# yzhang511/multi_modal_foundation_model

Measured on AMD Instinct MI355X. Metric: pretrain samples/sec (T=100 bins/modality, d_model=256, 5+5 layers, spike+behaviour masked pretraining step), higher is better.
Workload: dtype bf16; 1 GPU; BASELINE.json configs[1]: 1 session, ap(668 neurons)+behaviour(2), d_model=256, heads=8, mlp=512, 5 enc + 5 dec layers, T=100 (L=200 tokens), dropout 0.4/0.2, AdamW+OneCycleLR, mixed objectives; per_gpu_batch=1024, global_batch=1024, seq_len=200, parallelism=dp1

## Files before the change

### multi_modal_foundation_model_amd/csrc/attention_fast.hip

```cpp
#include "attn_common.h"
#include "attn_route.h"
#include <algorithm>
#include <stdlib.h>

using namespace attn;

namespace {

constexpr int KEEP_BITS = 10;

struct KeepArgs {
    uint32_t* bits;
    const uint32_t* state;
    uint32_t site, thresh;
    uint32_t nwords;
    int nkt, Lk;
};
__global__ __launch_bounds__(256) void attn_keepbits_kernel(const KeepArgs a) {
    const uint32_t gid = blockIdx.x * 256u + threadIdx.x;
    if (gid >= a.nwords) return;
    const uint32_t w = gid & 31u, kt = (gid >> 5) % (uint32_t)a.nkt;
    if ((int)(32u * kt + ((w >> 1) & 3u) + 8u * (w >> 3) + 4u * (w & 1u)) >= a.Lk) return;
    const uint32_t k0 = mix32(a.state[0] + a.site * 0x9E3779B9u), k1 = mix32(a.state[1] ^ (a.site * 0x85EBCA6Bu + 0xC2B2AE35u));
    const uint32_t s = mix32(gid ^ k0);
    const uint32_t kb = k1 + __umul24(s >> 24, 0x9E3779u);
    uint32_t r = 0;
#pragma unroll
    for (int j = 0; j < KEEP_BITS; ++j) {
        if ((a.thresh & ((2u << j) - 1u)) == 0) continue;
        uint32_t h = __umul24(s + (uint32_t)j * 0x3C6EF35Fu, 0x7FEB35u) + kb;
        h ^= h >> 13;
        h = __umul24(h, 0x46CA6Bu);
        h ^= h >> 16;
        r = ((a.thresh >> j) & 1u) ? (h | r) : (h & r);
    }
    a.bits[gid] = r;
}

__device__ __forceinline__ void stage_mod(uint8_t* modb, int* tmod, int t, int LP, uint32_t mv) {
    const int lane = t & 63;
    if (t < LP) modb[t] = (uint8_t)mv;
    const uint32_t first = (uint32_t)__shfl((int)mv, lane & 32);
    const uint64_t eq = __ballot(mv == first);
    const uint32_t half = (lane & 32) ? (uint32_t)(eq >> 32) : (uint32_t)eq;
    if ((lane & 31) == 0 && (t >> 5) < 8) tmod[t >> 5] = half == 0xffffffffu ? (int)mv : TMOD_MIXED;
}
template <int G, bool DROP>
__device__ __forceinline__ void fwd_tile(const f32x16& st, float c2, float nm, float& l_run, f32x16& acc, const Masks16& mk, const char* Vs,
                                         int kt, int lane) {
    uint32_t pk[8];
    float ps0 = 0.f, ps1 = 0.f;
#pragma unroll
    for (int r = 0; r < 16; r += 2) {
        if (r < 4 * G) {
            float p0 = __builtin_amdgcn_exp2f(__builtin_fmaf(st[r], c2, nm));
            float p1 = __builtin_amdgcn_exp2f(__builtin_fmaf(st[r + 1], c2, nm));
            ps0 = v_add(ps0, p0);
            ps1 = v_add(ps1, p1);
            if (DROP) {
                p0 = v_keep(p0, mk.m[r]);
                p1 = v_keep(p1, mk.m[r + 1]);
            }
            asm volatile("" : "+v"(p0), "+v"(p1), "+v"(ps0), "+v"(ps1));
            pk[r >> 1] = pack2(p0, p1);
        } else {
            pk[r >> 1] = 0u;
        }
    }
    l_run = v_add(l_run, v_add(ps0, ps1));
    const uint4 lo = make_uint4(pk[0], pk[1], pk[2], pk[3]), hi = make_uint4(pk[4], pk[5], pk[6], pk[7]);
    acc = __builtin_amdgcn_mfma_f32_32x32x16_bf16(trfrag(Vs, 64, kt * 32, 0, lane), __builtin_bit_cast(bf16x8v, lo), acc, 0, 0, 0);
    if (G > 2) acc = __builtin_amdgcn_mfma_f32_32x32x16_bf16(trfrag(Vs, 64, kt * 32 + 16, 0, lane), __builtin_bit_cast(bf16x8v, hi), acc, 0, 0, 0);
}
template <int G>
__device__ __forceinline__ float tile_max(const f32x16& st) {
    float mx = fmaxf(fmaxf(st[0], st[1]), st[2]);
#pragma unroll
    for (int r = 3; r < 4 * G; ++r) mx = fmaxf(mx, st[r]);
    return xhalf_max(mx);
}

constexpr int F_KRS = 80, F_VRS = 64, F_ORS = 80, F_MAXKT = 7;
constexpr float F_OVERFLOW = 1.2676506e30f;

template <int NW, bool DROP, int NKT, bool MASKED>
__global__ __launch_bounds__(NW * 64, 4) void attn_fwd_fast_kernel(const mmfm_attn_desc d, const float keep_scale) {
    constexpr int NT = NW * 64;
    extern __shared__ __attribute__((aligned(16))) char smem[];
    const int t = threadIdx.x, lane = t & 63, kh = lane >> 5, l31 = lane & 31;
    const int wave = __builtin_amdgcn_readfirstlane(t >> 6);
    const int bh_ = attn_xcd_remap((int)blockIdx.x, (int)gridDim.x, d.flags);
    const int b = bh_ / d.heads, h = bh_ % d.heads;
    const int Lq = d.Lq, Lk = d.Lk, LkP = NKT ? NKT * 32 : (Lk + 31) & ~31;
    const int nqt = (Lq + 31) >> 5, nkt = NKT ? NKT : LkP >> 5;
    char* Ks = smem;
    char* Vs = Ks + LkP * F_KRS;
    float* kbias = reinterpret_cast<float*>(Vs + LkP * F_VRS);
    char* ost = reinterpret_cast<char*>(kbias + LkP);
    int* wflag = reinterpret_cast<int*>(ost + NW * 32 * F_ORS);
    int* tmod = wflag + 8;
    float* kzero = reinterpret_cast<float*>(wflag + 16);
    uint8_t* modb = reinterpret_cast<uint8_t*>(kzero + LkP);
    const bool causal = MASKED && (d.flags & MMFM_ATTN_CAUSAL), sep = MASKED && (d.flags & MMFM_ATTN_SEP);
    const uint16_t* qg = reinterpret_cast<const uint16_t*>(d.q) + (size_t)b * Lq * d.ldq + h * 32;
    const uint16_t* kg = reinterpret_cast<const uint16_t*>(d.k) + (size_t)b * Lk * d.ldk + h * 32;
    const uint16_t* vg = reinterpret_cast<const uint16_t*>(d.v) + (size_t)b * Lk * d.ldv + h * 32;

    const int qt = wave;
    const int q0 = qt * 32, q = q0 + l31;
    uint4 kc[2], vc[2], qv[2];
    uint8_t kpv = 1;
#pragma unroll
    for (int j = 0; j < 2; ++j) {
        const int c = t + NT * j, row = c >> 2, col = c & 3;
        kc[j] = make_uint4(0u, 0u, 0u, 0u); vc[j] = kc[j];
        if (row < Lk) {
            kc[j] = *reinterpret_cast<const uint4*>(kg + (size_t)row * d.ldk + 8 * col);
            vc[j] = *reinterpret_cast<const uint4*>(vg + (size_t)row * d.ldv + 8 * col);
        }
    }
#pragma unroll
    for (int ks = 0; ks < 2; ++ks) {
        qv[ks] = make_uint4(0u, 0u, 0u, 0u);
        if (qt < nqt && q < Lq) qv[ks] = *reinterpret_cast<const uint4*>(qg + (size_t)q * d.ldq + ks * 16 + 8 * kh);
    }
    if (t < Lk && d.keypad != nullptr) kpv = d.keypad[(size_t)b * Lk + t];
    uint32_t mv = 0u;
    if constexpr (MASKED) {
        if (sep && t < LkP) mv = d.mod_id[min(t, Lk - 1)];
    }
#pragma unroll
    for (int j = 0; j < 2; ++j) {
        const int c = t + NT * j, row = c >> 2, col = c & 3;
        if (row < LkP) {
            *reinterpret_cast<uint4*>(Ks + row * F_KRS + col * 16) = kc[j];
            *reinterpret_cast<uint4*>(Vs + row * F_VRS + col * 16) = vc[j];
        }
    }
    const bool kok = t < Lk && (kpv != 0 || causal);
    if (t < LkP) kbias[t] = kok ? 0.f : -INFINITY;
    if constexpr (MASKED) {
        if (t < LkP) kzero[t] = t < Lk ? 0.f : -INFINITY;
        stage_mod(modb, tmod, t, LkP, mv);
    }
    const int pad = (t < Lk && !kok) ? 1 : 0;
    const int wv = __any(pad) ? 1 : 0;
    if (lane == 0) wflag[wave] = wv;
    __syncthreads();
    int anypad = 0;
#pragma unroll
    for (int w = 0; w < NW; ++w) anypad |= wflag[w];
    anypad = __builtin_amdgcn_readfirstlane(anypad);
    if (qt >= nqt) return;

    bf16x8v qf[2];
    qf[0] = __builtin_bit_cast(bf16x8v, qv[0]);
    qf[1] = __builtin_bit_cast(bf16x8v, qv[1]);
    const float c2 = d.scale * LOG2E;
    const bool fixdiag = anypad && (d.flags & MMFM_ATTN_DIAG);
    const masks_ptr mkp = reinterpret_cast<masks_ptr>(reinterpret_cast<uintptr_t>(d.keepbits)) + ((size_t)bh_ * nqt + qt) * nkt;
    int m_skip = 0, m_zero = 0, m_mix = 0, nkt_run = nkt;
    if constexpr (MASKED) {
        const int tq = sep ? tmod[qt] : 0;
        nkt_run = 1;
        for (int kt = 0; kt < nkt; ++kt) {
            const int c = tile_class(causal, sep, tq, sep ? tmod[kt] : 0, qt, kt);
            m_skip |= (c == T_SKIP) << kt;
            m_zero |= (c == T_ZERO) << kt;
            m_mix |= (c == T_MIXED) << kt;
            if (c != T_SKIP) nkt_run = kt + 1;
        }
        m_skip = __builtin_amdgcn_readfirstlane(m_skip);
        m_zero = __builtin_amdgcn_readfirstlane(m_zero);
        m_mix = __builtin_amdgcn_readfirstlane(m_mix);
        nkt_run = __builtin_amdgcn_readfirstlane(nkt_run);
    }
    auto skipped = [&](int kt) { return MASKED && ((m_skip >> kt) & 1); };

    auto score = [&](int kt) {
        const bool dfix = fixdiag && kt == qt;
        const float* bias = kbias;
        if constexpr (MASKED) bias = ((m_zero >> kt) & 1) ? kzero : kbias;
        f32x16 a;
#pragma unroll
        for (int g = 0; g < 4; ++g) {
            const float4 kb4 = *reinterpret_cast<const float4*>(bias + kt * 32 + 8 * g + 4 * kh);
            a[4 * g + 0] = kb4.x; a[4 * g + 1] = kb4.y; a[4 * g + 2] = kb4.z; a[4 * g + 3] = kb4.w;
        }
        if (dfix) {
            asm volatile("" ::: "memory");
#pragma unroll
            for (int r = 0; r < 16; ++r) a[r] = (mrow(r, kh) == l31) ? 0.f : a[r];
        }
        if constexpr (MASKED) {
            if ((m_mix >> kt) & 1) {
                asm volatile("" ::: "memory");
                const int fl = d.flags;
                const uint32_t mq = sep ? modb[q] : 0u;
#pragma unroll
                for (int g = 0; g < 4; ++g) {
                    const uint32_t mw = sep ? *reinterpret_cast<const uint32_t*>(modb + kt * 32 + 8 * g + 4 * kh) : 0u;
#pragma unroll
                    for (int i = 0; i < 4; ++i)
                        a[4 * g + i] = mixed_start(fl, q, kt * 32 + 8 * g + 4 * kh + i, Lk, a[4 * g + i], mq, (mw >> (8 * i)) & 0xffu);
                }
            }
        }
#pragma unroll
        for (int ks = 0; ks < 2; ++ks)
            a = __builtin_amdgcn_mfma_f32_32x32x16_bf16(rowfrag(Ks, (kt * 32 + l31) * F_KRS + ks * 32 + kh * 16), qf[ks], a, 0, 0, 0);
        return a;
    };
    const int gtail = ((Lk - (nkt - 1) * 32) + 7) >> 3;
    float m_ref, l_run = 0.f;
    f32x16 acc;
#pragma unroll
    for (int r = 0; r < 16; ++r) acc[r] = 0.f;
    auto tile = [&](int kt, const f32x16& st, const Masks16& mk) {
        if (kt == nkt - 1 && gtail != 4) {
            if (gtail == 1) fwd_tile<1, DROP>(st, c2, -m_ref, l_run, acc, mk, Vs, kt, lane);
            else if (gtail == 2) fwd_tile<2, DROP>(st, c2, -m_ref, l_run, acc, mk, Vs, kt, lane);
            else fwd_tile<3, DROP>(st, c2, -m_ref, l_run, acc, mk, Vs, kt, lane);
        } else {
            fwd_tile<4, DROP>(st, c2, -m_ref, l_run, acc, mk, Vs, kt, lane);
        }
    };
    {
        Masks16 mk[2];
        f32x16 sc[2];
        if (DROP) mk[0] = ld_masks(mkp);
        sc[0] = score(0);
        m_ref = v_max((nkt == 1 && gtail != 4) ? (gtail == 1 ? tile_max<1>(sc[0]) : gtail == 2 ? tile_max<2>(sc[0]) : tile_max<3>(sc[0]))
                                                : tile_max<4>(sc[0]), -1e30f / c2) * c2;
#pragma unroll
        for (int kt = 0; kt < F_MAXKT; ++kt) {
            if constexpr (!MASKED) {
                if (kt + 1 < nkt) {
                    sc[(kt + 1) & 1] = score(kt + 1);
                    if (DROP) mk[(kt + 1) & 1] = ld_masks(mkp + (kt + 1));
                }
                tile(kt, sc[kt & 1], mk[kt & 1]);
                if (kt + 1 >= nkt) break;
            } else {
                if (kt + 1 < nkt_run && !skipped(kt + 1)) {
                    sc[(kt + 1) & 1] = score(kt + 1);
                    if (DROP) mk[(kt + 1) & 1] = ld_masks(mkp + (kt + 1));
                }
                if (!skipped(kt)) tile(kt, sc[kt & 1], mk[kt & 1]);
                if (kt + 1 >= nkt_run) break;
            }
        }
    }
    float l_tot = xhalf_sum(l_run);
    if (__any(!(l_tot < F_OVERFLOW))) {
        float m_run = -1e30f;
        l_run = 0.f;
#pragma unroll
        for (int r = 0; r < 16; ++r) acc[r] = 0.f;
        for (int kt = 0; kt < nkt_run; ++kt) {
            if (skipped(kt)) continue;
            const f32x16 st = score(kt);
            Masks16 mk;
            if (DROP) mk = ld_masks(mkp + kt);
            const float mt = tile_max<4>(st) * c2;
            const float m_new = v_max(m_run, mt);
            const float alpha = __builtin_amdgcn_exp2f(m_run - m_new);
#pragma unroll
            for (int r = 0; r < 16; ++r) acc[r] *= alpha;
            l_run *= alpha;
            m_run = m_new;
            m_ref = m_run;
            tile(kt, st, mk);
        }
        l_tot = xhalf_sum(l_run);
    }
    const mmfm_attn_desc* kd = (const mmfm_attn_desc*)__builtin_amdgcn_kernarg_segment_ptr();
    asm volatile("" : "+s"(kd));
    const Drop dout = drop_init(kd->drop_o);
    const float inv = keep_scale / l_tot;
    if (kh == 0 && q < Lq) kd->lse[(size_t)bh_ * Lq + q] = m_ref * LN2 + __logf(l_tot);
    char* tl = ost + wave * 32 * F_ORS;
    const int heads = kd->heads, ldo = kd->ldo;
    uint16_t* og = reinterpret_cast<uint16_t*>(kd->o) + (size_t)b * Lq * ldo + h * 32;
    const uint64_t base = ((uint64_t)b * Lq + (uint64_t)q) * (uint64_t)(heads * 32) + (uint64_t)(h * 32);
#pragma unroll
    for (int g = 0; g < 4; ++g) {
        const int d0 = 8 * g + 4 * kh;
        float v0 = acc[4 * g + 0] * inv, v1 = acc[4 * g + 1] * inv, v2 = acc[4 * g + 2] * inv, v3 = acc[4 * g + 3] * inv;
        if (dout.on()) {
            dout.apply2(v0, v1, base + d0);
            dout.apply2(v2, v3, base + d0 + 2);
        }
        typedef __attribute__((ext_vector_type(4))) __bf16 bf16x4v;
        bf16x4v pk;
        pk[0] = (__bf16)v0; pk[1] = (__bf16)v1; pk[2] = (__bf16)v2; pk[3] = (__bf16)v3;
        *reinterpret_cast<uint2*>(tl + l31 * F_ORS + d0 * 2) = __builtin_bit_cast(uint2, pk);
    }
    wave_lds_fence();
#pragma unroll
    for (int i = 0; i < 2; ++i) {
        const int idx = lane + 64 * i, row = idx >> 2, c = idx & 3;
        if (q0 + row < Lq)
            *reinterpret_cast<uint4*>(og + (size_t)(q0 + row) * ldo + 8 * c) = *reinterpret_cast<const uint4*>(tl + row * F_ORS + c * 16);
    }
}

size_t fwd_fast_lds(int Lk, int nw, bool masked) {
    const int LkP = (Lk + 31) & ~31;
    return (size_t)LkP * (F_KRS + F_VRS + 4) + (size_t)nw * 32 * F_ORS + 64 + (masked ? (size_t)LkP * 5 : 0);
}

constexpr int B_NW = 8, B_CW = 7, B_TS = 80, B_TILE = 32 * B_TS, B_RS = 64, B_QRS = 80;

__device__ __forceinline__ int img_off(int row, int chunk) { return row * B_RS + ((chunk ^ ((row >> 2) & 3)) << 4); }
__device__ __forceinline__ bf16x8v trfrag_sw(const char* S, int rbase, int lane) {
    const int g = lane >> 4, li = lane & 15, q = li >> 2, p = li & 3;
    const int r0 = 4 * (g >> 1) + q;
    const int chunk = 2 * (g & 1) + (p >> 1), byte = 8 * (p & 1);
    const s16x4 lo = __builtin_amdgcn_ds_read_tr16_b64_v4i16((lds_s16x4*)(S + (rbase + r0) * B_RS + ((chunk ^ (g >> 1)) << 4) + byte));
    const s16x4 hi = __builtin_amdgcn_ds_read_tr16_b64_v4i16((lds_s16x4*)(S + (rbase + r0 + 8) * B_RS + ((chunk ^ ((g >> 1) + 2)) << 4) + byte));
    s16x8 v;
    v[0] = lo[0]; v[1] = lo[1]; v[2] = lo[2]; v[3] = lo[3]; v[4] = hi[0]; v[5] = hi[1]; v[6] = hi[2]; v[7] = hi[3];
    return __builtin_bit_cast(bf16x8v, v);
}

template <int GRP, bool DROP>
__device__ __forceinline__ void bwd_tile(const f32x16& s, const f32x16& dpv, float c2, const float* lse2, const float* dl, uint32_t wsh,
                                         const char* As, const char* Bs, char* slot, int qt, int kh, int lane, f32x16& dKt, f32x16& dVt) {
#pragma unroll
    for (int s2 = 0; s2 < 2; ++s2) {
        if (2 * s2 >= GRP) continue;
        const bool both = GRP > 2 * s2 + 1;
        float pd[8], ds[8];
        const int qb = qt * 32 + 16 * s2 + 4 * kh;
#pragma unroll
        for (int e4 = 0; e4 < 2; ++e4) {
            if (e4 == 1 && !both) {
#pragma unroll
                for (int e = 4; e < 8; ++e) { pd[e] = 0.f; ds[e] = 0.f; }
                continue;
            }
            const float4 l4 = *reinterpret_cast<const float4*>(lse2 + qb + 8 * e4), d4 = *reinterpret_cast<const float4*>(dl + qb + 8 * e4);
            const float lq[4] = {l4.x, l4.y, l4.z, l4.w}, dq_[4] = {d4.x, d4.y, d4.z, d4.w};
#pragma unroll
            for (int i = 0; i < 4; ++i) {
                const int e = 4 * e4 + i, r = 8 * s2 + e;
                const float p = __builtin_amdgcn_exp2f(__builtin_fmaf(s[r], c2, -lq[i]));
                float pm = p;
                if (DROP) {
                    int m = __builtin_amdgcn_sbfe((int)wsh, (r & 3) + 8 * (r >> 2), 1);
                    asm volatile("" : "+v"(m));
                    pm = __uint_as_float(__float_as_uint(p) & (uint32_t)m);
                }
                pd[e] = pm;
                ds[e] = __builtin_fmaf(pm, dpv[r], -v_mul(p, dq_[i]));
            }
        }
        const bf16x8v pf = pack8(pd), sf = pack8(ds);
        const uint4 sw = __builtin_bit_cast(uint4, sf);
        *reinterpret_cast<uint2*>(slot + (16 * s2 + 4 * kh) * 2) = make_uint2(sw.x, sw.y);
        *reinterpret_cast<uint2*>(slot + (16 * s2 + 8 + 4 * kh) * 2) = make_uint2(sw.z, sw.w);
        dVt = __builtin_amdgcn_mfma_f32_32x32x16_bf16(trfrag_sw(Bs, qt * 32 + 16 * s2, lane), pf, dVt, 0, 0, 0);
        dKt = __builtin_amdgcn_mfma_f32_32x32x16_bf16(trfrag_sw(As, qt * 32 + 16 * s2, lane), sf, dKt, 0, 0, 0);
    }
    if (GRP <= 2) {
        *reinterpret_cast<uint2*>(slot + (16 + 4 * kh) * 2) = make_uint2(0u, 0u);
        *reinterpret_cast<uint2*>(slot + (24 + 4 * kh) * 2) = make_uint2(0u, 0u);
    }
}

template <bool DROP, int NQT, bool MASKED>
__global__ __launch_bounds__(B_NW * 64, 4) void attn_bwd_fast_kernel(const mmfm_attn_desc d, const float keep_scale) {
    constexpr int NW = B_NW, CW = B_CW, TS = B_TS, TILE = B_TILE, RS = B_RS, NT = NW * 64;
    extern __shared__ __attribute__((aligned(16))) char smem[];
    const int t = threadIdx.x, lane = t & 63, kh = lane >> 5, l31 = lane & 31;
    const int wave = __builtin_amdgcn_readfirstlane(t >> 6);
    const int bh_ = attn_xcd_remap((int)blockIdx.x, (int)gridDim.x, d.flags);
    const int b = bh_ / d.heads, h = bh_ % d.heads;
    const int Lq = d.Lq, Lk = d.Lk, LqP = NQT ? NQT * 32 : (Lq + 31) & ~31, LkP = NQT ? NQT * 32 : (Lk + 31) & ~31;
    const int nqt = NQT ? NQT : LqP / 32, nkt = ((Lk + 31) & ~31) / 32;
    char* As = smem;
    char* Bs = As + LqP * RS;
    float* lse2 = reinterpret_cast<float*>(Bs + LqP * RS);
    float* dl = lse2 + LqP;
    float* kbias = dl + LqP;
    char* stg = reinterpret_cast<char*>(kbias + LkP);
    char* sc7 = stg + 2 * CW * TILE;
    uint32_t* flags = reinterpret_cast<uint32_t*>(sc7 + 32 * B_QRS);
    int* tmod = reinterpret_cast<int*>(flags + 8);
    uint8_t* modb = reinterpret_cast<uint8_t*>(flags + 16);
    const bool causal = MASKED && (d.flags & MMFM_ATTN_CAUSAL), sep = MASKED && (d.flags & MMFM_ATTN_SEP);
    const uint16_t* qg = reinterpret_cast<const uint16_t*>(d.q) + (size_t)b * Lq * d.ldq + h * 32;
    const uint16_t* kg = reinterpret_cast<const uint16_t*>(d.k) + (size_t)b * Lk * d.ldk + h * 32;
    const uint16_t* vg = reinterpret_cast<const uint16_t*>(d.v) + (size_t)b * Lk * d.ldv + h * 32;
    const uint16_t* og = reinterpret_cast<const uint16_t*>(d.o) + (size_t)b * Lq * d.ldo + h * 32;
    const uint16_t* dog = reinterpret_cast<const uint16_t*>(d.d_o) + (size_t)b * Lq * d.lddo + h * 32;
    const float osc_dk = d.scale * keep_scale, osc_dv = keep_scale, inv_keep = 1.f / keep_scale;
    const Drop dout = drop_init(d.drop_o);

    const int kt_own = wave < CW ? wave : 0, key_own = kt_own * 32 + l31;
    uint4 qc[2], kc[2], gc[2], oc[2], kfv[2], vfv[2];
#pragma unroll
    for (int j = 0; j < 2; ++j) {
        const int c = t + NT * j, row = c >> 2, col = c & 3;
        qc[j] = make_uint4(0u, 0u, 0u, 0u); kc[j] = qc[j]; gc[j] = qc[j]; oc[j] = qc[j];
        if (row < Lq) {
            qc[j] = *reinterpret_cast<const uint4*>(qg + (size_t)row * d.ldq + 8 * col);
            gc[j] = *reinterpret_cast<const uint4*>(dog + (size_t)row * d.lddo + 8 * col);
            oc[j] = *reinterpret_cast<const uint4*>(og + (size_t)row * d.ldo + 8 * col);
        }
        if (row < Lk) kc[j] = *reinterpret_cast<const uint4*>(kg + (size_t)row * d.ldk + 8 * col);
    }
#pragma unroll
    for (int ks = 0; ks < 2; ++ks) {
        kfv[ks] = make_uint4(0u, 0u, 0u, 0u); vfv[ks] = kfv[ks];
        if (wave < CW && key_own < Lk) {
            kfv[ks] = *reinterpret_cast<const uint4*>(kg + (size_t)key_own * d.ldk + ks * 16 + 8 * kh);
            vfv[ks] = *reinterpret_cast<const uint4*>(vg + (size_t)key_own * d.ldv + ks * 16 + 8 * kh);
        }
    }
    const uint32_t* kbp = reinterpret_cast<const uint32_t*>(d.keepbits) + ((size_t)bh_ * nqt * nkt + min(kt_own, nkt - 1)) * 32 +
                          2 * ((l31 & 3) + 4 * (l31 >> 3)) + ((l31 >> 2) & 1);
    const int kw_stride = nkt * 32;
    uint32_t kw_next = 0u;
    if (DROP) kw_next = kbp[0];
    float lsev = 0.f;
    uint8_t kpv = 1;
    if (t < Lq) lsev = d.lse[(size_t)bh_ * Lq + t];
    if (t < Lk && d.keypad != nullptr) kpv = d.keypad[(size_t)b * Lk + t];
    uint32_t mv = 0u;
    if constexpr (MASKED) {
        if (sep && t < LqP) mv = d.mod_id[min(t, Lq - 1)];
    }
#pragma unroll
    for (int j = 0; j < 2; ++j) {
        const int c = t + NT * j, row = c >> 2, col = c & 3;
        if (row < LqP) {
            *reinterpret_cast<uint4*>(As + img_off(row, col)) = qc[j];
            const uint32_t gw[4] = {gc[j].x, gc[j].y, gc[j].z, gc[j].w}, ow[4] = {oc[j].x, oc[j].y, oc[j].z, oc[j].w};
            const uint64_t base = ((uint64_t)b * Lq + (uint64_t)row) * (uint64_t)(d.heads * 32) + (uint64_t)(h * 32 + 8 * col);
            float part = 0.f, gd[8];
#pragma unroll
            for (int i = 0; i < 4; ++i) {
                float g0 = __uint_as_float(gw[i] << 16), g1 = __uint_as_float(gw[i] & 0xffff0000u);
                const float o0 = __uint_as_float(ow[i] << 16), o1 = __uint_as_float(ow[i] & 0xffff0000u);
                part += g0 * o0 + g1 * o1;
                if (dout.on()) dout.apply2(g0, g1, base + 2 * i);
                gd[2 * i] = g0;
                gd[2 * i + 1] = g1;
            }
            part += __shfl_xor(part, 1);
            part += __shfl_xor(part, 2);
            if (col == 0) dl[row] = part * inv_keep;
            *reinterpret_cast<uint4*>(Bs + img_off(row, col)) = __builtin_bit_cast(uint4, pack8(gd));
        }
        if (row < LkP) *reinterpret_cast<uint4*>(stg + img_off(row, col)) = kc[j];
    }
    if (t < LqP) lse2[t] = lsev * LOG2E;
    const bool kok = t < Lk && (kpv != 0 || causal);
    if (t < LkP) kbias[t] = kok ? 0.f : -INFINITY;
    if constexpr (MASKED) stage_mod(modb, tmod, t, LqP, mv);
    const int pad = (t < Lk && !kok) ? 1 : 0;
    const int wv = __any(pad) ? 1 : 0;
    if (lane == 0) flags[wave] = (uint32_t)wv;
    __syncthreads();
    int anypad = 0;
#pragma unroll
    for (int w = 0; w < NW; ++w) anypad |= (int)flags[w];
    anypad = __builtin_amdgcn_readfirstlane(anypad);
    const float c2 = d.scale * LOG2E;

    if (wave < CW) {
        const int kt = wave;
        const bool active = kt < nkt;
        f32x16 dKt, dVt;
#pragma unroll
        for (int r = 0; r < 16; ++r) { dKt[r] = 0.f; dVt[r] = 0.f; }
        const int key = kt * 32 + l31;
        bf16x8v kfr[2], vfr[2];
#pragma unroll
        for (int ks = 0; ks < 2; ++ks) {
            kfr[ks] = __builtin_bit_cast(bf16x8v, kfv[ks]);
            vfr[ks] = __builtin_bit_cast(bf16x8v, vfv[ks]);
        }
        const float kbv = active ? kbias[key] : 0.f;
        f32x16 s, dpv;
        int m_skip = 0, m_zero = 0, m_mix = 0;
        if constexpr (MASKED) {
            if (active) {
                const int tk = sep ? tmod[kt] : 0;
                for (int qt = 0; qt < nqt; ++qt) {
                    const int c = tile_class(causal, sep, sep ? tmod[qt] : 0, tk, qt, kt);
                    m_skip |= (c == T_SKIP) << qt;
                    m_zero |= (c == T_ZERO) << qt;
                    m_mix |= (c == T_MIXED) << qt;
                }
            }
            m_skip = __builtin_amdgcn_readfirstlane(m_skip);
            m_zero = __builtin_amdgcn_readfirstlane(m_zero);
            m_mix = __builtin_amdgcn_readfirstlane(m_mix);
        }
        const int roff0 = l31 * RS + (((0 + kh) ^ ((l31 >> 2) & 3)) << 4), roff1 = l31 * RS + (((2 + kh) ^ ((l31 >> 2) & 3)) << 4);
        auto scoresA = [&](int qt) {
            const char* Aq = As + qt * (32 * RS);
            const char* Bq = Bs + qt * (32 * RS);
            const f32x16 zero = {0.f, 0.f, 0.f, 0.f, 0.f, 0.f, 0.f, 0.f, 0.f, 0.f, 0.f, 0.f, 0.f, 0.f, 0.f, 0.f};
            bool zero_start = !anypad, mixed = false;
            if constexpr (MASKED) {
                zero_start = zero_start || ((m_zero >> qt) & 1);
                mixed = (m_mix >> qt) & 1;
            }
            if (mixed) {
                const int fl = d.flags;
                const uint32_t mk = sep ? modb[key] : 0u;
#pragma unroll
                for (int g = 0; g < 4; ++g) {
                    const uint32_t mw = sep ? *reinterpret_cast<const uint32_t*>(modb + qt * 32 + 8 * g + 4 * kh) : 0u;
#pragma unroll
                    for (int i = 0; i < 4; ++i)
                        s[4 * g + i] = mixed_start(fl, qt * 32 + 8 * g + 4 * kh + i, key, Lk, kbv, (mw >> (8 * i)) & 0xffu, mk);
                }
                s = __builtin_amdgcn_mfma_f32_32x32x16_bf16(rowfrag(Aq, roff0), kfr[0], s, 0, 0, 0);
                dpv = __builtin_amdgcn_mfma_f32_32x32x16_bf16(rowfrag(Bq, roff0), vfr[0], zero, 0, 0, 0);
                s = __builtin_amdgcn_mfma_f32_32x32x16_bf16(rowfrag(Aq, roff1), kfr[1], s, 0, 0, 0);
                dpv = __builtin_amdgcn_mfma_f32_32x32x16_bf16(rowfrag(Bq, roff1), vfr[1], dpv, 0, 0, 0);
            } else if (zero_start) {
                s = __builtin_amdgcn_mfma_f32_32x32x16_bf16(rowfrag(Aq, roff0), kfr[0], zero, 0, 0, 0);
                dpv = __builtin_amdgcn_mfma_f32_32x32x16_bf16(rowfrag(Bq, roff0), vfr[0], zero, 0, 0, 0);
                s = __builtin_amdgcn_mfma_f32_32x32x16_bf16(rowfrag(Aq, roff1), kfr[1], s, 0, 0, 0);
                dpv = __builtin_amdgcn_mfma_f32_32x32x16_bf16(rowfrag(Bq, roff1), vfr[1], dpv, 0, 0, 0);
            } else {
                const bool dfix = (d.flags & MMFM_ATTN_DIAG) && qt == kt;
                int lv = l31;
                asm volatile("" : "+v"(lv));
#pragma unroll
                for (int r = 0; r < 16; ++r) s[r] = (dfix && mrow(r, kh) == lv) ? 0.f : kbv;
                s = __builtin_amdgcn_mfma_f32_32x32x16_bf16(rowfrag(Aq, roff0), kfr[0], s, 0, 0, 0);
                dpv = __builtin_amdgcn_mfma_f32_32x32x16_bf16(rowfrag(Bq, roff0), vfr[0], zero, 0, 0, 0);
                s = __builtin_amdgcn_mfma_f32_32x32x16_bf16(rowfrag(Aq, roff1), kfr[1], s, 0, 0, 0);
                dpv = __builtin_amdgcn_mfma_f32_32x32x16_bf16(rowfrag(Bq, roff1), vfr[1], dpv, 0, 0, 0);
            }
        };
        const int gtail = ((Lq - (nqt - 1) * 32) + 7) >> 3;
        __syncthreads();
        auto step = [&](int qt) {
            bool skip = false;
            if constexpr (MASKED) skip = (m_skip >> qt) & 1;
            if (active && skip) {
                if (DROP) kw_next = kbp[(size_t)min(qt + 1, nqt - 1) * kw_stride];
                char* slot = stg + ((qt & 1) * CW + wave) * TILE + l31 * TS;
#pragma unroll
                for (int j = 0; j < 4; ++j) *reinterpret_cast<uint2*>(slot + (8 * j + 4 * kh) * 2) = make_uint2(0u, 0u);
            } else if (active) {
                scoresA(qt);
                uint32_t wq = 0u;
                if (DROP) {
                    wq = kw_next >> (4 * kh);
                    kw_next = kbp[(size_t)min(qt + 1, nqt - 1) * kw_stride];
                }
                char* slot = stg + ((qt & 1) * CW + wave) * TILE + l31 * TS;
                if (qt == nqt - 1 && gtail != 4) {
                    if (gtail == 1) bwd_tile<1, DROP>(s, dpv, c2, lse2, dl, wq, As, Bs, slot, qt, kh, lane, dKt, dVt);
                    else if (gtail == 2) bwd_tile<2, DROP>(s, dpv, c2, lse2, dl, wq, As, Bs, slot, qt, kh, lane, dKt, dVt);
                    else bwd_tile<3, DROP>(s, dpv, c2, lse2, dl, wq, As, Bs, slot, qt, kh, lane, dKt, dVt);
                } else {
                    bwd_tile<4, DROP>(s, dpv, c2, lse2, dl, wq, As, Bs, slot, qt, kh, lane, dKt, dVt);
                }
            }
            __syncthreads();
        };
        if constexpr (NQT != 0) {
#pragma unroll
            for (int qt = 0; qt < NQT; ++qt) step(qt);
        } else {
            for (int qt = 0; qt < nqt; ++qt) step(qt);
        }
        if (active) {
            char* scr = stg + ((nqt & 1) * CW + wave) * TILE;
            const f32x16 dk1[1] = {dKt}, dv1[1] = {dVt};
            store_tile_T<32, 1>(scr, TS, dk1, reinterpret_cast<uint16_t*>(d.dk) + (size_t)b * Lk * d.lddk + h * 32, d.lddk, kt * 32, Lk, lane, osc_dk);
            store_tile_T<32, 1>(scr, TS, dv1, reinterpret_cast<uint16_t*>(d.dv) + (size_t)b * Lk * d.lddv + h * 32, d.lddv, kt * 32, Lk, lane, osc_dv);
        }
    } else {
        bf16x8v kT[CW][2];
#pragma unroll
        for (int kt = 0; kt < CW; ++kt)
#pragma unroll
            for (int s2 = 0; s2 < 2; ++s2) kT[kt][s2] = trfrag_sw(stg, min(kt, nkt - 1) * 32 + 16 * s2, lane);
        __syncthreads();
        uint16_t* dqg = reinterpret_cast<uint16_t*>(d.dq) + (size_t)b * Lq * d.lddq + h * 32;
        auto step = [&](int qt) {
            __syncthreads();
            const char* buf = stg + (qt & 1) * CW * TILE;
            f32x16 dQt[1];
#pragma unroll
            for (int r = 0; r < 16; ++r) dQt[0][r] = 0.f;
#pragma unroll
            for (int kt = 0; kt < CW; ++kt) {
                if (kt < nkt) {
#pragma unroll
                    for (int s2 = 0; s2 < 2; ++s2)
                        dQt[0] = __builtin_amdgcn_mfma_f32_32x32x16_bf16(kT[kt][s2], trfrag(buf + kt * TILE, TS, 16 * s2, 0, lane), dQt[0], 0, 0, 0);
                }
            }
            store_tile_T<32, 1>(sc7, B_QRS, dQt, dqg, d.lddq, qt * 32, Lq, lane, osc_dk);
        };
        if constexpr (NQT != 0) {
#pragma unroll
            for (int qt = 0; qt < NQT; ++qt) step(qt);
        } else {
            for (int qt = 0; qt < nqt; ++qt) step(qt);
        }
    }
}

size_t bwd_fast_lds(int Lq, int Lk, bool masked) {
    const int LqP = (Lq + 31) & ~31, LkP = (Lk + 31) & ~31;
    return (size_t)2 * LqP * B_RS + (size_t)2 * LqP * 4 + (size_t)LkP * 4 + (size_t)2 * B_CW * B_TILE + (size_t)32 * B_QRS + 64 +
           (masked ? (size_t)LqP : 0);
}

}

static uint32_t keep_thresh(float p) {
    const int one = 1 << KEEP_BITS;
    const int t = (int)lrintf((1.f - p) * (float)one);
    return (uint32_t)std::min(std::max(t, 1), one - 1);
}
extern "C" float mmfm_attn_keep_prob(float p) { return p <= 0.f ? 1.f : (float)keep_thresh(p) / (float)(1 << KEEP_BITS); }
extern "C" int64_t mmfm_attn_keepbits_bytes(int B, int heads, int Lq, int Lk) {
    const int64_t tiles = (int64_t)B * heads * ((Lq + 31) / 32) * ((Lk + 31) / 32) * 128;
    return tiles + (((int64_t)B * heads * Lq * 4 + 127) & ~(int64_t)127);
}

int mmfm_attn_keepbits_launch(const mmfm_attn_desc& d, hipStream_t st) {
    KeepArgs a;
    a.bits = reinterpret_cast<uint32_t*>(d.keepbits);
    a.state = reinterpret_cast<const uint32_t*>(d.drop_p.state);
    a.site = d.drop_p.site;
    a.thresh = keep_thresh(d.drop_p.p);
    a.nkt = (d.Lk + 31) / 32;
    a.Lk = d.Lk;
    a.nwords = (uint32_t)((int64_t)d.B * d.heads * ((d.Lq + 31) / 32) * a.nkt * 32);
    hipLaunchKernelGGL(attn_keepbits_kernel, dim3((a.nwords + 255) / 256), dim3(256), 0, st, a);
    MMFM_LAUNCH_CHECK("mmfm_attn_fwd(keep bits)");
    return 0;
}

bool mmfm_attn_fast_takes(const mmfm_attn_desc& d) {
    static const bool off = [] { const char* e = getenv("MMFM_ATTN_FAST"); return e && atoi(e) == 0; }();
    if (off || d.dh != 32) return false;
    const bool masked = (d.flags & (MMFM_ATTN_CAUSAL | MMFM_ATTN_SEP)) != 0;
    if (masked && (d.Lq != d.Lk || ((d.flags & MMFM_ATTN_SEP) && d.mod_id == nullptr))) return false;
    const int nqt = (d.Lq + 31) / 32, nkt = (d.Lk + 31) / 32;
    if (d.Lq % 8 || d.Lk % 8 || nqt > 8 || nkt > B_CW || nkt > nqt) return false;
    const bool drop = attn_drop_p_on(d);
    if (drop && d.drop_p.p >= 1.f) return false;
    if (drop && d.keepbits == nullptr) return false;
    return attn_io_aligned(d) && (uintptr_t)d.keepbits % 128 == 0;
}

int mmfm_attn_fast_launch(const mmfm_attn_desc& d, bool backward, hipStream_t st) {
    const bool masked = (d.flags & (MMFM_ATTN_CAUSAL | MMFM_ATTN_SEP)) != 0, drop = attn_drop_p_on(d);
    const int nqt = (d.Lq + 31) / 32, nkt = (d.Lk + 31) / 32;
    const int grid = d.B * d.heads;
    const float keep_scale = drop ? 1.f / mmfm_attn_keep_prob(d.drop_p.p) : 1.f;
    if (!backward) {
        if (drop) { if (int rc = mmfm_attn_keepbits_launch(d, st)) return rc; }
        const int nw = nqt <= 4 ? 4 : (nqt == 7 ? 7 : (nqt <= 6 ? 6 : 8));
        const size_t lds = fwd_fast_lds(d.Lk, nw, masked);
#define FWDF4(NWV, DRP, NKT, MSK)                                                                                   \
        {                                                                                                           \
            auto kern = attn_fwd_fast_kernel<NWV, DRP, NKT, MSK>;                                                   \
            if (int rc = mmfm_lds_opt_in(reinterpret_cast<const void*>(kern), lds, "mmfm_attn_fwd(bf16, dh 32)")) return rc; \
            hipLaunchKernelGGL(kern, dim3(grid), dim3(NWV * 64), lds, st, d, keep_scale);                           \
        }
#define FWDF3(NWV, DRP, NKT) { if (masked) FWDF4(NWV, DRP, NKT, true) else FWDF4(NWV, DRP, NKT, false) }
#define FWDF(NWV)                                                                                                   \
        {                                                                                                           \
            if (drop) { if (nkt == 7 && NWV >= 7) FWDF3(NWV, true, 7) else FWDF3(NWV, true, 0) }                    \
            else { if (nkt == 7 && NWV >= 7) FWDF3(NWV, false, 7) else FWDF3(NWV, false, 0) }                       \
        }
        if (nw == 4) FWDF(4) else if (nw == 6) FWDF(6) else if (nw == 7) FWDF(7) else FWDF(8)
#undef FWDF
#undef FWDF3
#undef FWDF4
        MMFM_LAUNCH_CHECK("mmfm_attn_fwd(bf16, dh 32)");
        return 0;
    }
    const size_t lds = nqt == 7 ? bwd_fast_lds(224, 224, masked) : bwd_fast_lds(d.Lq, d.Lk, masked);
#define BWDF4(DRP, NQ, MSK)                                                                                         \
    {                                                                                                               \
        auto kern = attn_bwd_fast_kernel<DRP, NQ, MSK>;                                                             \
        if (int rc = mmfm_lds_opt_in(reinterpret_cast<const void*>(kern), lds, "mmfm_attn_bwd(bf16, dh 32)")) return rc; \
        hipLaunchKernelGGL(kern, dim3(grid), dim3(B_NW * 64), lds, st, d, keep_scale);                              \
    }
#define BWDF3(DRP, NQ) { if (masked) BWDF4(DRP, NQ, true) else BWDF4(DRP, NQ, false) }
    if (drop) { if (nqt == 7) BWDF3(true, 7) else BWDF3(true, 0) }
    else { if (nqt == 7) BWDF3(false, 7) else BWDF3(false, 0) }
#undef BWDF3
#undef BWDF4
    MMFM_LAUNCH_CHECK("mmfm_attn_bwd(bf16, dh 32)");
    return 0;
}
```

Measured before the change: 35570 samples/s.

## Re-layout attention backward dS staging tile and use LDS-typed pointers

Changes the shared-memory staging layout for the dS tile in the attention backward kernel. Rows are no longer padded at 80 bytes; the tile is grouped by query in 288-byte strides and read back with transpose loads. It precomputes per-lane LDS address-space pointers so the hot loop only adds constant offsets. It also adds a permlane32-swap based transposed tile store with a swizzled layout, replacing the generic padded store. The aim is fewer address computations and bank conflicts, plus a smaller scratch area, at the cost of more intricate indexing that must stay consistent between the dK/dV and dQ waves.

```diff
diff --git a/multi_modal_foundation_model_amd/csrc/attention_fast.hip b/multi_modal_foundation_model_amd/csrc/attention_fast.hip
--- a/multi_modal_foundation_model_amd/csrc/attention_fast.hip
+++ b/multi_modal_foundation_model_amd/csrc/attention_fast.hip
@@ -310,23 +310,74 @@
     return (size_t)LkP * (F_KRS + F_VRS + 4) + (size_t)nw * 32 * F_ORS + 64 + (masked ? (size_t)LkP * 5 : 0);
 }
 
-constexpr int B_NW = 8, B_CW = 7, B_TS = 80, B_TILE = 32 * B_TS, B_RS = 64, B_QRS = 80;
+constexpr int B_NW = 8, B_CW = 7, B_SP = 288, B_TILE = 8 * B_SP, B_RS = 64, B_TT = 32 * 64;
 
 __device__ __forceinline__ int img_off(int row, int chunk) { return row * B_RS + ((chunk ^ ((row >> 2) & 3)) << 4); }
-__device__ __forceinline__ bf16x8v trfrag_sw(const char* S, int rbase, int lane) {
+__device__ __forceinline__ void trfrag_sw_offs(int lane, int& lo, int& hi) {
     const int g = lane >> 4, li = lane & 15, q = li >> 2, p = li & 3;
     const int r0 = 4 * (g >> 1) + q;
     const int chunk = 2 * (g & 1) + (p >> 1), byte = 8 * (p & 1);
-    const s16x4 lo = __builtin_amdgcn_ds_read_tr16_b64_v4i16((lds_s16x4*)(S + (rbase + r0) * B_RS + ((chunk ^ (g >> 1)) << 4) + byte));
-    const s16x4 hi = __builtin_amdgcn_ds_read_tr16_b64_v4i16((lds_s16x4*)(S + (rbase + r0 + 8) * B_RS + ((chunk ^ ((g >> 1) + 2)) << 4) + byte));
+    lo = r0 * B_RS + ((chunk ^ (g >> 1)) << 4) + byte;
+    hi = (r0 + 8) * B_RS + ((chunk ^ ((g >> 1) + 2)) << 4) + byte;
+}
+typedef __attribute__((address_space(3))) char lds_char;
+typedef const __attribute__((address_space(3))) uint4 lds_cuint4;
+typedef __attribute__((ext_vector_type(2))) uint32_t u32x2;
+typedef __attribute__((address_space(3))) u32x2 lds_u32x2;
+__device__ __forceinline__ bf16x8v rowfrag_lds(const lds_char* p, int off) { return __builtin_bit_cast(bf16x8v, *(lds_cuint4*)(p + off)); }
+__device__ __forceinline__ bf16x8v trfrag_sw_at(const lds_char* plo, const lds_char* phi, int off) {
+    const s16x4 lo = __builtin_amdgcn_ds_read_tr16_b64_v4i16((lds_s16x4*)(plo + off));
+    const s16x4 hi = __builtin_amdgcn_ds_read_tr16_b64_v4i16((lds_s16x4*)(phi + off));
     s16x8 v;
     v[0] = lo[0]; v[1] = lo[1]; v[2] = lo[2]; v[3] = lo[3]; v[4] = hi[0]; v[5] = hi[1]; v[6] = hi[2]; v[7] = hi[3];
     return __builtin_bit_cast(bf16x8v, v);
 }
+__device__ __forceinline__ bf16x8v trfrag_sw(const char* S, int rbase, int lane) {
+    int lo, hi;
+    trfrag_sw_offs(lane, lo, hi);
+    return trfrag_sw_at((const lds_char*)(S + lo), (const lds_char*)(S + hi), rbase * B_RS);
+}
+
+__device__ __forceinline__ int stg_off(int key, int qg) { return qg * B_SP + key * 8; }
+__device__ __forceinline__ bf16x8v trfrag_stg(const char* T, int rbase, int lane) {
+    const int g = lane >> 4, li = lane & 15, q = li >> 2, p = li & 3;
+    const int key = rbase + 4 * (g >> 1) + q, qg = 4 * (g & 1) + p;
+    const s16x4 lo = __builtin_amdgcn_ds_read_tr16_b64_v4i16((lds_s16x4*)(T + stg_off(key, qg)));
+    const s16x4 hi = __builtin_amdgcn_ds_read_tr16_b64_v4i16((lds_s16x4*)(T + stg_off(key + 8, qg)));
+    s16x8 v;
+    v[0] = lo[0]; v[1] = lo[1]; v[2] = lo[2]; v[3] = lo[3]; v[4] = hi[0]; v[5] = hi[1]; v[6] = hi[2]; v[7] = hi[3];
+    return __builtin_bit_cast(bf16x8v, v);
+}
+
+__device__ __forceinline__ int tt_off(int row, int chunk) { return row * 64 + ((chunk ^ ((row >> 1) & 3)) << 4); }
+__device__ __forceinline__ void store_tile_T32(char* tile, const f32x16& acc, uint16_t* outg, int ld, int row0, int nrows_total, int lane,
+                                               float osc) {
+    const int l31 = lane & 31, kh = lane >> 5;
+    uint32_t w[4][2];
+#pragma unroll
+    for (int g = 0; g < 4; ++g) {
+        w[g][0] = pack2(acc[4 * g + 0] * osc, acc[4 * g + 1] * osc);
+        w[g][1] = pack2(acc[4 * g + 2] * osc, acc[4 * g + 3] * osc);
+    }
+    wave_lds_fence();
+#pragma unroll
+    for (int gp = 0; gp < 2; ++gp) {
+        const auto x = __builtin_amdgcn_permlane32_swap(w[2 * gp][0], w[2 * gp + 1][0], false, false);
+        const auto y = __builtin_amdgcn_permlane32_swap(w[2 * gp][1], w[2 * gp + 1][1], false, false);
+        *reinterpret_cast<uint4*>(tile + tt_off(l31, 2 * gp + kh)) = make_uint4(x[0], y[0], x[1], y[1]);
+    }
+    wave_lds_fence();
+#pragma unroll
+    for (int j = 0; j < 2; ++j) {
+        const int idx = lane + 64 * j, row = idx >> 2, c = idx & 3;
+        if (row0 + row < nrows_total)
+            *reinterpret_cast<uint4*>(outg + (size_t)(row0 + row) * ld + 8 * c) = *reinterpret_cast<const uint4*>(tile + tt_off(row, c));
+    }
+}
 
 template <int GRP, bool DROP>
 __device__ __forceinline__ void bwd_tile(const f32x16& s, const f32x16& dpv, float c2, const float* lse2, const float* dl, uint32_t wsh,
-                                         const char* As, const char* Bs, char* slot, int qt, int kh, int lane, f32x16& dKt, f32x16& dVt) {
+                                         const lds_char* tlo, const lds_char* thi, int bs_off, lds_char* slot, int qt, int kh, f32x16& dKt, f32x16& dVt) {
 #pragma unroll
     for (int s2 = 0; s2 < 2; ++s2) {
         if (2 * s2 >= GRP) continue;
@@ -358,20 +409,20 @@
         }
         const bf16x8v pf = pack8(pd), sf = pack8(ds);
         const uint4 sw = __builtin_bit_cast(uint4, sf);
-        *reinterpret_cast<uint2*>(slot + (16 * s2 + 4 * kh) * 2) = make_uint2(sw.x, sw.y);
-        *reinterpret_cast<uint2*>(slot + (16 * s2 + 8 + 4 * kh) * 2) = make_uint2(sw.z, sw.w);
-        dVt = __builtin_amdgcn_mfma_f32_32x32x16_bf16(trfrag_sw(Bs, qt * 32 + 16 * s2, lane), pf, dVt, 0, 0, 0);
-        dKt = __builtin_amdgcn_mfma_f32_32x32x16_bf16(trfrag_sw(As, qt * 32 + 16 * s2, lane), sf, dKt, 0, 0, 0);
+        *(lds_u32x2*)(slot + stg_off(0, 4 * s2)) = u32x2{sw.x, sw.y};
+        *(lds_u32x2*)(slot + stg_off(0, 4 * s2 + 2)) = u32x2{sw.z, sw.w};
+        dVt = __builtin_amdgcn_mfma_f32_32x32x16_bf16(trfrag_sw_at(tlo, thi, bs_off + (qt * 32 + 16 * s2) * B_RS), pf, dVt, 0, 0, 0);
+        dKt = __builtin_amdgcn_mfma_f32_32x32x16_bf16(trfrag_sw_at(tlo, thi, (qt * 32 + 16 * s2) * B_RS), sf, dKt, 0, 0, 0);
     }
     if (GRP <= 2) {
-        *reinterpret_cast<uint2*>(slot + (16 + 4 * kh) * 2) = make_uint2(0u, 0u);
-        *reinterpret_cast<uint2*>(slot + (24 + 4 * kh) * 2) = make_uint2(0u, 0u);
+        *(lds_u32x2*)(slot + stg_off(0, 4)) = u32x2{0u, 0u};
+        *(lds_u32x2*)(slot + stg_off(0, 6)) = u32x2{0u, 0u};
     }
 }
 
 template <bool DROP, int NQT, bool MASKED>
 __global__ __launch_bounds__(B_NW * 64, 4) void attn_bwd_fast_kernel(const mmfm_attn_desc d, const float keep_scale) {
-    constexpr int NW = B_NW, CW = B_CW, TS = B_TS, TILE = B_TILE, RS = B_RS, NT = NW * 64;
+    constexpr int NW = B_NW, CW = B_CW, TILE = B_TILE, RS = B_RS, NT = NW * 64;
     extern __shared__ __attribute__((aligned(16))) char smem[];
     const int t = threadIdx.x, lane = t & 63, kh = lane >> 5, l31 = lane & 31;
     const int wave = __builtin_amdgcn_readfirstlane(t >> 6);
@@ -386,7 +437,7 @@
     float* kbias = dl + LqP;
     char* stg = reinterpret_cast<char*>(kbias + LkP);
     char* sc7 = stg + 2 * CW * TILE;
-    uint32_t* flags = reinterpret_cast<uint32_t*>(sc7 + 32 * B_QRS);
+    uint32_t* flags = reinterpret_cast<uint32_t*>(sc7 + B_TT);
     int* tmod = reinterpret_cast<int*>(flags + 8);
     uint8_t* modb = reinterpret_cast<uint8_t*>(flags + 16);
     const bool causal = MASKED && (d.flags & MMFM_ATTN_CAUSAL), sep = MASKED && (d.flags & MMFM_ATTN_SEP);
@@ -419,11 +470,14 @@
             vfv[ks] = *reinterpret_cast<const uint4*>(vg + (size_t)key_own * d.ldv + ks * 16 + 8 * kh);
         }
     }
-    const uint32_t* kbp = reinterpret_cast<const uint32_t*>(d.keepbits) + ((size_t)bh_ * nqt * nkt + min(kt_own, nkt - 1)) * 32 +
-                          2 * ((l31 & 3) + 4 * (l31 >> 3)) + ((l31 >> 2) & 1);
+    const uint32_t* kbu = reinterpret_cast<const uint32_t*>(d.keepbits) + ((size_t)bh_ * nqt * nkt + min(kt_own, nkt - 1)) * 32;
+    const uint32_t kbl = 4u * (uint32_t)(2 * ((l31 & 3) + 4 * (l31 >> 3)) + ((l31 >> 2) & 1));
     const int kw_stride = nkt * 32;
+    auto kw_load = [&](int qt) -> uint32_t {
+        return *reinterpret_cast<const uint32_t*>(reinterpret_cast<const char*>(kbu + (size_t)qt * kw_stride) + kbl);
+    };
     uint32_t kw_next = 0u;
-    if (DROP) kw_next = kbp[0];
+    if (DROP) kw_next = kw_load(0);
     float lsev = 0.f;
     uint8_t kpv = 1;
     if (t < Lq) lsev = d.lse[(size_t)bh_ * Lq + t];
@@ -500,10 +554,17 @@
             m_zero = __builtin_amdgcn_readfirstlane(m_zero);
             m_mix = __builtin_amdgcn_readfirstlane(m_mix);
         }
-        const int roff0 = l31 * RS + (((0 + kh) ^ ((l31 >> 2) & 3)) << 4), roff1 = l31 * RS + (((2 + kh) ^ ((l31 >> 2) & 3)) << 4);
+        const lds_char* roff0 = (const lds_char*)(As + l31 * RS + (((0 + kh) ^ ((l31 >> 2) & 3)) << 4));
+        const lds_char* roff1 = (const lds_char*)(As + l31 * RS + (((2 + kh) ^ ((l31 >> 2) & 3)) << 4));
+        int tlo_, thi_;
+        trfrag_sw_offs(lane, tlo_, thi_);
+        const lds_char* tlo = (const lds_char*)(As + tlo_);
+        const lds_char* thi = (const lds_char*)(As + thi_);
+        lds_char* slot_l = (lds_char*)(stg + wave * TILE + stg_off(l31, kh));
+        asm volatile("" : "+v"(roff0), "+v"(roff1), "+v"(tlo), "+v"(thi), "+v"(slot_l));
+        const int bs_off = LqP * RS;
         auto scoresA = [&](int qt) {
-            const char* Aq = As + qt * (32 * RS);
-            const char* Bq = Bs + qt * (32 * RS);
+            const int Aq = qt * (32 * RS), Bq = bs_off + qt * (32 * RS);
             const f32x16 zero = {0.f, 0.f, 0.f, 0.f, 0.f, 0.f, 0.f, 0.f, 0.f, 0.f, 0.f, 0.f, 0.f, 0.f, 0.f, 0.f};
             bool zero_start = !anypad, mixed = false;
             if constexpr (MASKED) {
@@ -520,25 +581,25 @@
                     for (int i = 0; i < 4; ++i)
                         s[4 * g + i] = mixed_start(fl, qt * 32 + 8 * g + 4 * kh + i, key, Lk, kbv, (mw >> (8 * i)) & 0xffu, mk);
                 }
-                s = __builtin_amdgcn_mfma_f32_32x32x16_bf16(rowfrag(Aq, roff0), kfr[0], s, 0, 0, 0);
-                dpv = __builtin_amdgcn_mfma_f32_32x32x16_bf16(rowfrag(Bq, roff0), vfr[0], zero, 0, 0, 0);
-                s = __builtin_amdgcn_mfma_f32_32x32x16_bf16(rowfrag(Aq, roff1), kfr[1], s, 0, 0, 0);
-                dpv = __builtin_amdgcn_mfma_f32_32x32x16_bf16(rowfrag(Bq, roff1), vfr[1], dpv, 0, 0, 0);
+                s = __builtin_amdgcn_mfma_f32_32x32x16_bf16(rowfrag_lds(roff0, Aq), kfr[0], s, 0, 0, 0);
+                dpv = __builtin_amdgcn_mfma_f32_32x32x16_bf16(rowfrag_lds(roff0, Bq), vfr[0], zero, 0, 0, 0);
+                s = __builtin_amdgcn_mfma_f32_32x32x16_bf16(rowfrag_lds(roff1, Aq), kfr[1], s, 0, 0, 0);
+                dpv = __builtin_amdgcn_mfma_f32_32x32x16_bf16(rowfrag_lds(roff1, Bq), vfr[1], dpv, 0, 0, 0);
             } else if (zero_start) {
-                s = __builtin_amdgcn_mfma_f32_32x32x16_bf16(rowfrag(Aq, roff0), kfr[0], zero, 0, 0, 0);
-                dpv = __builtin_amdgcn_mfma_f32_32x32x16_bf16(rowfrag(Bq, roff0), vfr[0], zero, 0, 0, 0);
-                s = __builtin_amdgcn_mfma_f32_32x32x16_bf16(rowfrag(Aq, roff1), kfr[1], s, 0, 0, 0);
-                dpv = __builtin_amdgcn_mfma_f32_32x32x16_bf16(rowfrag(Bq, roff1), vfr[1], dpv, 0, 0, 0);
+                s = __builtin_amdgcn_mfma_f32_32x32x16_bf16(rowfrag_lds(roff0, Aq), kfr[0], zero, 0, 0, 0);
+                dpv = __builtin_amdgcn_mfma_f32_32x32x16_bf16(rowfrag_lds(roff0, Bq), vfr[0], zero, 0, 0, 0);
+                s = __builtin_amdgcn_mfma_f32_32x32x16_bf16(rowfrag_lds(roff1, Aq), kfr[1], s, 0, 0, 0);
+                dpv = __builtin_amdgcn_mfma_f32_32x32x16_bf16(rowfrag_lds(roff1, Bq), vfr[1], dpv, 0, 0, 0);
             } else {
                 const bool dfix = (d.flags & MMFM_ATTN_DIAG) && qt == kt;
                 int lv = l31;
                 asm volatile("" : "+v"(lv));
 #pragma unroll
                 for (int r = 0; r < 16; ++r) s[r] = (dfix && mrow(r, kh) == lv) ? 0.f : kbv;
-                s = __builtin_amdgcn_mfma_f32_32x32x16_bf16(rowfrag(Aq, roff0), kfr[0], s, 0, 0, 0);
-                dpv = __builtin_amdgcn_mfma_f32_32x32x16_bf16(rowfrag(Bq, roff0), vfr[0], zero, 0, 0, 0);
-                s = __builtin_amdgcn_mfma_f32_32x32x16_bf16(rowfrag(Aq, roff1), kfr[1], s, 0, 0, 0);
-                dpv = __builtin_amdgcn_mfma_f32_32x32x16_bf16(rowfrag(Bq, roff1), vfr[1], dpv, 0, 0, 0);
+                s = __builtin_amdgcn_mfma_f32_32x32x16_bf16(rowfrag_lds(roff0, Aq), kfr[0], s, 0, 0, 0);
+                dpv = __builtin_amdgcn_mfma_f32_32x32x16_bf16(rowfrag_lds(roff0, Bq), vfr[0], zero, 0, 0, 0);
+                s = __builtin_amdgcn_mfma_f32_32x32x16_bf16(rowfrag_lds(roff1, Aq), kfr[1], s, 0, 0, 0);
+                dpv = __builtin_amdgcn_mfma_f32_32x32x16_bf16(rowfrag_lds(roff1, Bq), vfr[1], dpv, 0, 0, 0);
             }
         };
         const int gtail = ((Lq - (nqt - 1) * 32) + 7) >> 3;
@@ -547,24 +608,24 @@
             bool skip = false;
             if constexpr (MASKED) skip = (m_skip >> qt) & 1;
             if (active && skip) {
-                if (DROP) kw_next = kbp[(size_t)min(qt + 1, nqt - 1) * kw_stride];
-                char* slot = stg + ((qt & 1) * CW + wave) * TILE + l31 * TS;
-#pragma unroll
-                for (int j = 0; j < 4; ++j) *reinterpret_cast<uint2*>(slot + (8 * j + 4 * kh) * 2) = make_uint2(0u, 0u);
+                if (DROP) kw_next = kw_load(min(qt + 1, nqt - 1));
+                lds_char* slot = slot_l + (qt & 1) * (CW * TILE);
+#pragma unroll
+                for (int j = 0; j < 4; ++j) *(lds_u32x2*)(slot + stg_off(0, 2 * j)) = u32x2{0u, 0u};
             } else if (active) {
                 scoresA(qt);
                 uint32_t wq = 0u;
                 if (DROP) {
                     wq = kw_next >> (4 * kh);
-                    kw_next = kbp[(size_t)min(qt + 1, nqt - 1) * kw_stride];
-                }
-                char* slot = stg + ((qt & 1) * CW + wave) * TILE + l31 * TS;
+                    kw_next = kw_load(min(qt + 1, nqt - 1));
+                }
+                lds_char* slot = slot_l + (qt & 1) * (CW * TILE);
                 if (qt == nqt - 1 && gtail != 4) {
-                    if (gtail == 1) bwd_tile<1, DROP>(s, dpv, c2, lse2, dl, wq, As, Bs, slot, qt, kh, lane, dKt, dVt);
-                    else if (gtail == 2) bwd_tile<2, DROP>(s, dpv, c2, lse2, dl, wq, As, Bs, slot, qt, kh, lane, dKt, dVt);
-                    else bwd_tile<3, DROP>(s, dpv, c2, lse2, dl, wq, As, Bs, slot, qt, kh, lane, dKt, dVt);
+                    if (gtail == 1) bwd_tile<1, DROP>(s, dpv, c2, lse2, dl, wq, tlo, thi, bs_off, slot, qt, kh, dKt, dVt);
+                    else if (gtail == 2) bwd_tile<2, DROP>(s, dpv, c2, lse2, dl, wq, tlo, thi, bs_off, slot, qt, kh, dKt, dVt);
+                    else bwd_tile<3, DROP>(s, dpv, c2, lse2, dl, wq, tlo, thi, bs_off, slot, qt, kh, dKt, dVt);
                 } else {
-                    bwd_tile<4, DROP>(s, dpv, c2, lse2, dl, wq, As, Bs, slot, qt, kh, lane, dKt, dVt);
+                    bwd_tile<4, DROP>(s, dpv, c2, lse2, dl, wq, tlo, thi, bs_off, slot, qt, kh, dKt, dVt);
                 }
             }
             __syncthreads();
@@ -577,9 +638,8 @@
         }
         if (active) {
             char* scr = stg + ((nqt & 1) * CW + wave) * TILE;
-            const f32x16 dk1[1] = {dKt}, dv1[1] = {dVt};
-            store_tile_T<32, 1>(scr, TS, dk1, reinterpret_cast<uint16_t*>(d.dk) + (size_t)b * Lk * d.lddk + h * 32, d.lddk, kt * 32, Lk, lane, osc_dk);
-            store_tile_T<32, 1>(scr, TS, dv1, reinterpret_cast<uint16_t*>(d.dv) + (size_t)b * Lk * d.lddv + h * 32, d.lddv, kt * 32, Lk, lane, osc_dv);
+            store_tile_T32(scr, dKt, reinterpret_cast<uint16_t*>(d.dk) + (size_t)b * Lk * d.lddk + h * 32, d.lddk, kt * 32, Lk, lane, osc_dk);
+            store_tile_T32(scr, dVt, reinterpret_cast<uint16_t*>(d.dv) + (size_t)b * Lk * d.lddv + h * 32, d.lddv, kt * 32, Lk, lane, osc_dv);
         }
     } else {
         bf16x8v kT[CW][2];
@@ -592,18 +652,18 @@
         auto step = [&](int qt) {
             __syncthreads();
             const char* buf = stg + (qt & 1) * CW * TILE;
-            f32x16 dQt[1];
-#pragma unroll
-            for (int r = 0; r < 16; ++r) dQt[0][r] = 0.f;
+            f32x16 dQt;
+#pragma unroll
+            for (int r = 0; r < 16; ++r) dQt[r] = 0.f;
 #pragma unroll
             for (int kt = 0; kt < CW; ++kt) {
                 if (kt < nkt) {
 #pragma unroll
                     for (int s2 = 0; s2 < 2; ++s2)
-                        dQt[0] = __builtin_amdgcn_mfma_f32_32x32x16_bf16(kT[kt][s2], trfrag(buf + kt * TILE, TS, 16 * s2, 0, lane), dQt[0], 0, 0, 0);
-                }
-            }
-            store_tile_T<32, 1>(sc7, B_QRS, dQt, dqg, d.lddq, qt * 32, Lq, lane, osc_dk);
+                        dQt = __builtin_amdgcn_mfma_f32_32x32x16_bf16(kT[kt][s2], trfrag_stg(buf + kt * TILE, 16 * s2, lane), dQt, 0, 0, 0);
+                }
+            }
+            store_tile_T32(sc7, dQt, dqg, d.lddq, qt * 32, Lq, lane, osc_dk);
         };
         if constexpr (NQT != 0) {
 #pragma unroll
@@ -616,7 +676,7 @@
 
 size_t bwd_fast_lds(int Lq, int Lk, bool masked) {
     const int LqP = (Lq + 31) & ~31, LkP = (Lk + 31) & ~31;
-    return (size_t)2 * LqP * B_RS + (size_t)2 * LqP * 4 + (size_t)LkP * 4 + (size_t)2 * B_CW * B_TILE + (size_t)32 * B_QRS + 64 +
+    return (size_t)2 * LqP * B_RS + (size_t)2 * LqP * 4 + (size_t)LkP * 4 + (size_t)2 * B_CW * B_TILE + (size_t)B_TT + 64 +
            (masked ? (size_t)LqP : 0);
 }
 
```

Result: no change. 35780 samples/s (median of 6 runs) (+0.6%).
